# AsteriosPar/mmWave_MSc

Measured on AMD Instinct MI355X. Metric: scene_frames_per_sec, higher is better.
Workload: dtype f64

## Files before the change

mmwave_msc_amd/csrc/api_context.hip:

```cpp
#include <cmath>
#include <cstdarg>
#include <cstdio>
#include <new>

#include "mmw_ctx.hpp"
#include "mmw_kalman.hpp"

thread_local LaunchProf mmw::g_launch_prof;

static thread_local std::string g_last_error;

int fail(mmw_ctx *ctx, int code, const char *fmt, ...)
{
    char buf[512];
    va_list ap;
    va_start(ap, fmt);
    vsnprintf(buf, sizeof(buf), fmt, ap);
    va_end(ap);
    if (ctx) ctx->err = buf;
    g_last_error = buf;
    return code;
}

constexpr int kPerSceneMaxScenes = 512;
constexpr int kSideWorkerMinScenes = kPerSceneMaxScenes + 1;

static hipError_t create_side_streams(mmw_ctx *c)
{
    hipError_t e = hipStreamCreateWithFlags(&c->side_stream, hipStreamNonBlocking);
    if (e == hipSuccess) e = hipEventCreateWithFlags(&c->side_gate, hipEventDisableTiming);
    return e;
}

static int probe_one(mmw_ctx *c, hipStream_t side, hipStream_t other)
{
    const int polls = 1 << 12;
    if (hipMemsetAsync(c->d_probe, 0, 4 * sizeof(int32_t), c->stream) != hipSuccess || hipStreamSynchronize(c->stream) != hipSuccess) return -1;
    launch_probe_wait(c->d_probe, 0, polls, side);
    launch_probe_set(c->d_probe, other);
    if (hipStreamSynchronize(side) != hipSuccess || hipStreamSynchronize(other) != hipSuccess) return -1;
    int32_t w[4] = {0, 0, 0, 0};
    if (hipMemcpy(w, c->d_probe, sizeof(w), hipMemcpyDeviceToHost) != hipSuccess) return -1;
    return w[1] ? 1 : 0;
}
int probe_side_streams(mmw_ctx *c)
{
    int ok = probe_one(c, c->side_stream, c->stream);
    for (int attempt = 0; ok == 0 && attempt < 6; attempt++) {
        hipStream_t fresh = nullptr;
        if (hipStreamCreateWithFlags(&fresh, hipStreamNonBlocking) != hipSuccess) return -1;
        hipStreamSynchronize(c->side_stream);
        hipStreamDestroy(c->side_stream);
        c->side_stream = fresh;
        ok = probe_one(c, fresh, c->stream);
    }
    return ok;
}

static int check_create_args(const mmw_config *cfg, int32_t n_scenes, int32_t max_pts)
{
    if (n_scenes < 1 || max_pts < 1 || max_pts > MMW_MAX_PTS_LIMIT) return fail(nullptr, MMW_E_ARG, "mmw_create: n_scenes=%d max_pts=%d out of range (max_pts <= %d)", n_scenes, max_pts, MMW_MAX_PTS_LIMIT);
    if (cfg->fb_frames_batch < 0 || cfg->fb_frames_batch + 1 > MMW_RING_MAX) return fail(nullptr, MMW_E_ARG, "FB_FRAMES_BATCH must be in [0,%d]", MMW_RING_MAX - 1);
    if (cfg->dim_x != 9 && cfg->dim_x != 6) return fail(nullptr, MMW_E_ARG, "dim_x must be 9 (CONST_ACC_MODEL) or 6 (CONST_VEL_MODEL)");
    if (!(cfg->db_eps > 0.0) || cfg->db_min_samples < 1 || (cfg->seek_inner && !(cfg->db_inner_eps > 0.0)))
        return fail(nullptr, MMW_E_ARG, "DB_EPS%s must be > 0 and DB_MIN_SAMPLES_MIN >= 1 (sklearn's DBSCAN refuses anything else)", cfg->seek_inner ? " / DB_INNER_EPS" : "");
    const int um = (cfg->fb_frames_batch + 1) * max_pts;
    if (um > MMW_RING_MAX * MMW_MAX_PTS_LIMIT) return fail(nullptr, MMW_E_ARG, "ring*max_pts = %d exceeds %d", um, MMW_RING_MAX * MMW_MAX_PTS_LIMIT);
    return MMW_OK;
}

struct DevPlan { DevCfg dc; int fused_wanted, side_wanted, side_trusted, gate_side; };
static int derive_dev_cfg(const mmw_config *cfg, int32_t n_scenes, int32_t max_pts, DevPlan &plan)
{
    DevCfg &d = plan.dc;
    memset(&d, 0, sizeof(d));
    const int ring = cfg->fb_frames_batch + 1;
    d.ring = ring; d.db_min_samples = cfg->db_min_samples; d.tr_max_tracks = cfg->tr_max_tracks;
    d.kf_enable_est = cfg->kf_enable_est; d.model_min_input = cfg->model_min_input; d.dx = cfg->dim_x;
    d.ring_rows = cfg->ring_rows < 64 ? 64 : cfg->ring_rows;
    d.seek_inner = cfg->seek_inner ? 1 : 0;
    d.db_points_thres = cfg->db_points_thres; d.fb_frames_batch_static = cfg->fb_frames_batch_static;
    d.db_spread_thres = cfg->db_spread_thres; d.db_inner_eps = cfg->db_inner_eps;
    d.side_worker = (!d.seek_inner && (cfg->chain_side_stream > 0 || (cfg->chain_side_stream == 0 && n_scenes >= kSideWorkerMinScenes))) ? 1 : 0;
    if (d.seek_inner) {
        if (cfg->fb_frames_batch < 1 || cfg->fb_frames_batch_static < 1 || cfg->fb_frames_batch_static > ring)
            return fail(nullptr, MMW_E_ARG, "seek_inner: FB_FRAMES_BATCH and FB_FRAMES_BATCH_STATIC must be in [1, FB_FRAMES_BATCH + 1 = %d]", ring);
        if (d.ring_rows < ring * max_pts) d.ring_rows = ring * max_pts;
    }
    int cap = cfg->track_cap;
    if (cap <= 0) {
        const int ms = cfg->db_min_samples > 0 ? cfg->db_min_samples : 1;
        cap = (cfg->tr_max_tracks > 0 ? cfg->tr_max_tracks - 1 : 0) + (ring * max_pts) / ms + 1;
    }
    if (cap > MMW_TRACK_CAP_LIMIT) cap = MMW_TRACK_CAP_LIMIT;
    if (cap < 1) cap = 1;
    d.t_cap = cap; d.max_pts = max_pts; d.n_scenes = n_scenes;
    d.dense_min_units = cfg->kalman_dense_min_units == 0 ? (n_scenes <= kPerSceneMaxScenes ? 0x7fffffff : 1024)
                                                         : (cfg->kalman_dense_min_units < 0 ? 0x7fffffff : cfg->kalman_dense_min_units - 1);
    if (d.seek_inner) d.dense_min_units = 0x7fffffff;
    d.db_z_weight = cfg->db_z_weight; d.db_range_weight = cfg->db_range_weight; d.db_eps = cfg->db_eps;
    d.tr_lifetime_dynamic = cfg->tr_lifetime_dynamic; d.tr_lifetime_static = cfg->tr_lifetime_static;
    d.tr_vel_thres = cfg->tr_vel_thres; d.tr_gate = cfg->tr_gate; d.kf_q_std = cfg->kf_q_std; d.kf_p_init = cfg->kf_p_init;
    d.kf_group_disp_est_init = cfg->kf_group_disp_est_init; d.kf_a_n = cfg->kf_a_n; d.kf_est_pointnum = cfg->kf_est_pointnum;
    for (int i = 0; i < 6; i++) d.kf_spread_lim[i] = cfg->kf_spread_lim[i];
    d.kf_a_spr = cfg->kf_a_spr; d.intensity_mu = cfg->intensity_mu; d.intensity_std = cfg->intensity_std;
    d.s_height = cfg->s_height; d.tilt_cos = cfg->tilt_cos; d.tilt_sin = cfg->tilt_sin;
    d.m_x = cfg->m_x; d.m_y = cfg->m_y; d.m_z = cfg->m_z;
    d.fade_max = cfg->v_screen_fade_size_max; d.fade_min = cfg->v_screen_fade_size_min; d.fade_weight = cfg->v_screen_fade_weight;
    const size_t sl = scene_lds_bytes(d);
    const int per_cu = (sl <= 80 * 1024 && max_pts <= 512) ? 2 : (sl <= 160 * 1024 ? 1 : 0);
    const bool can = per_cu > 0 && !d.seek_inner && d.t_cap <= 63 && cfg->chain_side_stream <= 0;
    const bool want = cfg->fused_step > 0 || (cfg->fused_step == 0 && cfg->kalman_dense_min_units == 0 && n_scenes <= 256 * per_cu && n_scenes <= kPerSceneMaxScenes);
    plan.fused_wanted = d.fused = (can && want) ? 1 : 0;
    if (d.fused) { d.dense_min_units = 0x7fffffff; d.side_worker = 0; }
    plan.side_wanted = d.side_worker;
    plan.side_trusted = (d.side_worker && cfg->chain_side_stream == 2) ? 1 : 0;
    plan.gate_side = (d.side_worker && cfg->chain_side_stream == 3) ? 1 : 0;
    return MMW_OK;
}

static size_t trk_bytes(const DevCfg &d) { return (size_t)d.n_scenes * d.t_cap * sizeof(TrackRec); }
static size_t db_list_bytes(const DevCfg &d) { return 4 * (size_t)d.n_scenes * sizeof(int32_t); }
static size_t upd_list_bytes(const DevCfg &d) { return 2 * (size_t)kUpdShards * upd_region(d.n_scenes, d.t_cap) * sizeof(int32_t); }
static size_t inner_buf_bytes(const mmw_ctx *c) { return (size_t)c->dc.n_scenes * (size_t)(kInnerHdr + c->st.inner_cap) * sizeof(int32_t); }
constexpr size_t kStatAllocBytes = kStatBytes + (256 + 8192) * sizeof(unsigned long long);
constexpr size_t kDbCountBytes = 8 * sizeof(int32_t), kQBytes = kQWords * sizeof(int32_t), kSpcCountBytes = 2 * sizeof(int32_t), kUpdCountBytes = 2 * kUpdWords * sizeof(int32_t);

#define CREATE_FAIL(c, ...) do { mmw_destroy(c); return fail(nullptr, __VA_ARGS__); } while (0)

static int create_alloc(mmw_ctx *c)
{
    const DevCfg &d = c->dc;
#ifdef MMW_DIAG_POISON
#define MMW_POISON_FRESH(ptr, bytes) (void)hipMemsetAsync((void *)(ptr), 0xFF, (bytes), c->own_stream)
#else
#define MMW_POISON_FRESH(ptr, bytes) ((void)0)
#endif
    if (hipStreamCreateWithFlags(&c->own_stream, hipStreamNonBlocking) != hipSuccess) CREATE_FAIL(c, MMW_E_HIP, "hipStreamCreate failed");
    c->stream = c->own_stream;
#define ALLOC(ptr, bytes)                                                                                   \
    do {                                                                                                    \
        hipError_t e_ = hipMalloc((void **)&(ptr), (bytes));                                                \
        if (e_ != hipSuccess) { int rc = fail(nullptr, MMW_E_HIP, "hipMalloc(%zu) -> %s", (size_t)(bytes), hipGetErrorString(e_)); mmw_destroy(c); return rc; } \
        MMW_POISON_FRESH(ptr, bytes);                                                                       \
    } while (0)
    const size_t S = (size_t)d.n_scenes, cap = (size_t)d.t_cap;
    ALLOC(c->st.hdr, S * sizeof(SceneHdr));
    ALLOC(c->st.order, S * cap * sizeof(int32_t));
    ALLOC(c->st.trk, trk_bytes(d));
    ALLOC(c->st.trk_ring, S * cap * (size_t)d.ring * d.ring_rows * 8 * sizeof(double));
    ALLOC(c->st.g_ring, S * (size_t)d.ring * d.max_pts * 8 * sizeof(double));
    ALLOC(c->d_posture, MMW_NKP * sizeof(float));
    ALLOC(c->d_row_off, (S + 1) * sizeof(int32_t));
    ALLOC(c->st.stats, kStatAllocBytes);
    ALLOC(c->st.db_list, db_list_bytes(d));
    ALLOC(c->st.db_count, kDbCountBytes);
    ALLOC(c->st.q, kQBytes);
    ALLOC(c->d_probe, 4 * sizeof(int32_t));
    ALLOC(c->st.gate_buf, S * cap * kGateRec * sizeof(double));
    ALLOC(c->st.perm, 2 * S * sizeof(int32_t));
    ALLOC(c->st.upd_count, kUpdCountBytes);
    ALLOC(c->st.upd_list, upd_list_bytes(d));
    ALLOC(c->st.spc_count, kSpcCountBytes);
    ALLOC(c->st.spc_list, 4 * S * sizeof(int32_t));
    if (d.seek_inner) {
        c->st.inner_cap = 2 * inner_um(d);
        ALLOC(c->st.inner_buf, inner_buf_bytes(c));
    }
#undef ALLOC
#undef MMW_POISON_FRESH
    c->st.default_posture = c->d_posture;
    return MMW_OK;
}

static int create_init_device(mmw_ctx *c, int32_t n_scenes)
{
    const DevCfg &d = c->dc;
    const mmw_config *cfg = &c->cfg;
#ifdef MMW_MUTANT_NULL_STREAM_INIT
#define MMW_FILL0(ptr, bytes) hipMemset((ptr), 0, (bytes))
#else
#define MMW_FILL0(ptr, bytes) hipMemsetAsync((ptr), 0, (bytes), c->own_stream)
#endif
    if (hipMemcpyAsync(c->d_posture, cfg->default_posture, MMW_NKP * sizeof(float), hipMemcpyHostToDevice, c->own_stream) != hipSuccess ||
// ... 384 lines not shown
```

mmwave_msc_amd/csrc/k_track.hip:

```cpp
#include <cstdlib>

#include "mmw_device.hpp"
#include "mmw_math.hpp"
#include "mmw_cloud.hpp"
#include "mmw_kalman.hpp"
#include "mmw_assoc.hpp"
#include "mmw_launch.hpp"
#include "mmw_kernels.hpp"

namespace mmw {

#ifdef MMW_STAMPS
#define STAMP(k)                                                                              \
    do {                                                                                      \
        if (tid == 0) {                                                                       \
            const unsigned long long t_now = __builtin_amdgcn_s_memtime();                   \
            atomicAdd(&stats_slot(st, blockIdx.x)[8 + (k)], t_now - t_prev);                                    \
            t_prev = t_now;                                                                   \
        }                                                                                     \
    } while (0)
#else
#define STAMP(k)
#endif

struct TrackLds {
    double *p6;
    double *work;
    double *cen;
    unsigned short *cnt;
    int *cls_n;
    int *cls_off;
    long long *seg_dst;
    double *wmm;
    double *nest;
    int *ml;
    int *slot;
    int *slot2;
    int *misc;
};

template <bool WRITE>
__host__ __device__ __forceinline__ size_t track_lds_layout(const DevCfg &c, char *base, TrackLds *L)
{
    const int NP = c.max_pts, NB = (NP + 63) / 64, CLS = c.t_cap + 1;
    const int work_a = 0, work_b = 6 * (NP + kTilePad) + pw_max_leaves(NP) * 21;
    size_t off = 0;
#define CARVE(field, type, count)                            \
    if constexpr (WRITE) L->field = (type *)(base + off);    \
    off = align16(off + sizeof(type) * (size_t)(count));
    if constexpr (WRITE) L->p6 = (double *)(base + off);
    const int work_c = (12288 + 256 * 4 + 64) / 8;
    const int work_ab = work_a > work_b ? work_a : work_b;
    CARVE(work, double, work_ab > work_c ? work_ab : work_c)
    CARVE(cen, double, c.t_cap * 6)
    {
        const size_t base_off = off;
        CARVE(cnt, unsigned short, NB *CLS)
        CARVE(seg_dst, long long, CLS + 1)
        const size_t end_a = off;
        off = base_off;
        CARVE(wmm, double, kWaves * 24)
        CARVE(nest, double, c.t_cap)
        CARVE(slot2, int, c.t_cap)
        off = off > end_a ? off : end_a;
    }
    CARVE(cls_n, int, CLS)
    CARVE(cls_off, int, CLS + 1)
    CARVE(ml, int, ml_words(NP))
    CARVE(slot, int, c.t_cap)
    CARVE(misc, int, 16)
#undef CARVE
    return off;
}

size_t track_lds_bytes(const DevCfg &c)
{
    size_t b = track_lds_layout<false>(c, nullptr, nullptr);
    if (pred_in_track(c) && b < (size_t)16 * kPredScratch * sizeof(double)) b = (size_t)16 * kPredScratch * sizeof(double);
#ifdef MMW_STAMPS
    if (const char *x = getenv("MMW_DIAG_LDS_EXTRA")) b += (size_t)atoi(x);
#endif
    return b;
}

template <int PPT, bool INNER, bool PRED = false, bool F32 = false>
__global__ __launch_bounds__(kThreads, (PRED ? 2 : (PPT == 2 ? 5 : (PPT == 1 ? 4 : 3)))) void k_track(DevCfg cfg, DevState st, const void *__restrict__ pts_all,
                                                    const int32_t *__restrict__ n_pts, const double *__restrict__ dt_all,
                                                    int32_t *__restrict__ assoc_out, int32_t *__restrict__ db_n_out,
                                                    int32_t *__restrict__ db_labels_out, int UM_out, int parity)
{
    extern __shared__ __attribute__((aligned(16))) char lds_raw[];
    TrackLds L;
    track_lds_layout<true>(cfg, lds_raw, &L);

    const int s = st.perm[(size_t)parity * cfg.n_scenes + blockIdx.x];
    const int tid = threadIdx.x;
    const int lane = tid & 63, wave = tid >> 6;
    PROBE(19);
    WGTIME(0);
    const int role = (wave + s) & (kWaves - 1);
    const int NP = cfg.max_pts, CLS = cfg.t_cap + 1;
    const int NPs = NP + kTilePad;
    const int my_slot = tid < cfg.t_cap ? st.order[(size_t)s * cfg.t_cap + tid] : 0;
    const int n_raw = n_pts[s];
    SceneHdr *hdr = st.hdr + s;
    const double dt = dt_all[s];
    int T = hdr->n_tracks;
    double2 pr[PPT][4];
    {
        const void *frame = frame_of(pts_all, s, NP, F32);
#pragma unroll
        for (int q = 0; q < PPT; q++) {
            const int i = q * kThreads + tid;
            load_point_row<F32>(frame, i, i < NP, pr[q]);
        }
    }
    const int n = n_raw < 0 ? 0 : n_raw;
    if (tid == 0 && db_n_out) db_n_out[s] = -1;
    if (s == 0 && tid < 4) st.db_count[(parity ^ 1) * 4 + tid] = 0;
    if (s == 0 && tid >= 4 && tid < 7) st.q[(parity ^ 1) * 8 + (tid - 4)] = tid - 4 == kQHead ? q_tag(cfg.epoch + 1) : 0;
    if (s == 0 && tid >= 8 && tid < 11) st.q[kQBig + (parity ^ 1) * 8 + (tid - 8)] = tid - 8 == kQHead ? q_tag(cfg.epoch + 1) : 0;
    if (s == 0 && tid < kUpdWords) st.upd_count[(parity ^ 1) * kUpdWords + tid] = 0;
    if (s == 0 && tid == kThreads - 1) st.spc_count[parity ^ 1] = 0;
    if (!frame_reaches_track(n_raw, NP)) {
        if (tid == 0) frame_skipped(hdr, hdr->skipped, n_raw);
        return;
    }
    int32_t *order = st.order + (size_t)s * cfg.t_cap;
    TrackRec *trk = st.trk + (size_t)s * cfg.t_cap;
    const int Tin = T;
    int err = 0;
#ifdef MMW_STAMPS
    unsigned long long t_prev = __builtin_amdgcn_s_memtime();
#endif
    PROBE(16);
    if constexpr (PRED) {
        double *Wj = reinterpret_cast<double *>(lds_raw) + (size_t)(wave * 4 + (lane >> 4)) * kPredScratch;
        int perr = 0;
        for (int j0 = wave * 4; j0 < T; j0 += 4 * kWaves) {
            const int j = j0 + (lane >> 4);
            const bool live = j < T;
            TrackRec *rec = trk + (live ? order[j] : 0);
            if (cfg.dx == 9) predict_one_track<9>(cfg, st, rec, live, s, j, dt, Wj, lane, lane & 15, perr);
            else predict_one_track<6>(cfg, st, rec, live, s, j, dt, Wj, lane, lane & 15, perr);
        }
        PROBE(17);
        if (perr) atomicOr(&hdr->err, perr);
        __builtin_amdgcn_s_waitcnt(0x0F70);
        __builtin_amdgcn_fence(__ATOMIC_RELEASE, "workgroup");
        __syncthreads();
        __builtin_amdgcn_s_dcache_inv();
        __builtin_amdgcn_s_waitcnt(0xC07F);
        PROBE(18);
    }

    if (tid < cfg.t_cap) L.slot[tid] = my_slot;
    for (int j = tid + kThreads; j < cfg.t_cap; j += kThreads) L.slot[j] = order[j];
    if (tid == 0) { L.ml[0] = 0; L.ml[1] = 0; L.misc[15] = 0; }
    lds_barrier();
    STAMP(0);
    PROBE(0);

    double bestd[PPT];
    int bestj[PPT];
#pragma unroll
    for (int q = 0; q < PPT; q++) { bestd[q] = 0.0; bestj[q] = -1; }

    {
        const int su = __builtin_amdgcn_readfirstlane(s), Tu = __builtin_amdgcn_readfirstlane(T);
        gate_ptr gb = (gate_ptr)(st.gate_buf + (size_t)su * cfg.t_cap * kGateRec);
        if constexpr (PRED) {
            gb = gate_records_opaque(gb);
#ifndef MMW_DIAG_VGATE
            typedef const int __attribute__((address_space(4))) *line_ptr;
            const unsigned long long a0 = (unsigned long long)gb & ~63ULL;
            const int lines = (int)((((unsigned long long)gb + (unsigned long long)Tu * kGateRec * 8 + 63ULL) & ~63ULL) - a0) >> 6;
            line_ptr w = (line_ptr)a0;
            int acc = 0;
            for (int l0 = 0; l0 < lines; l0 += 16) {
                int t[16];
#pragma unroll
                for (int u = 0; u < 16; u++) { const int l = l0 + u < lines ? l0 + u : lines - 1; t[u] = w[l * 16]; }
#pragma unroll
                for (int u = 0; u < 16; u++) acc |= t[u];
            }
            asm volatile("" : : "s"(acc));
#endif
        }
        PROBE(32);
        for (int j = 0; j < Tu; j++) {
            if (j < 8) PROBE(33 + j);
            gate_ptr G = gb + j * kGateRec;
#pragma unroll
            for (int q = 0; q < PPT; q++) {
                const int i = q * kThreads + tid;
                if (q * kThreads < n) {
                    const double d = gate_distance(G, pr[q][0].x, pr[q][0].y, pr[q][1].x, pr[q][1].y, pr[q][2].x, pr[q][2].y);
                    gate_first_best(cfg, i < n, d, j, bestj[q], bestd[q]);
                }
            }
        }
    }
    STAMP(1);
    STAMP(2);
    PROBE(2);
    int gp_len, gp_skw, gp_s[MMW_RING_MAX], gp_n[MMW_RING_MAX];
    {
        const int NB = (n + 63) / 64;
        unsigned long long mybal[PPT];
        int sd_len = 0, sd_rs[MMW_RING_MAX] = {0, 0, 0, 0}, sd_size = cfg.ring;
        gp_len = 0; gp_skw = 0;
#pragma unroll
        for (int k = 0; k < MMW_RING_MAX; k++) { gp_s[k] = 0; gp_n[k] = 0; }
        if (tid < T) {
            const TrackRec *rec = trk + L.slot[tid];
            sd_len = rec->ring_len;
            if (INNER) sd_size = rec->inner & 255;
#pragma unroll
            for (int k = 0; k < MMW_RING_MAX; k++) sd_rs[k] = rec->ring_slot[k];
        } else if (tid == T) {
            sd_len = hdr->g_len;
            if (INNER && hdr_ring_size(hdr->skipped)) sd_size = hdr_ring_size(hdr->skipped);
#pragma unroll
            for (int k = 0; k < MMW_RING_MAX; k++) sd_rs[k] = hdr->g_slot[k];
        } else if (tid == kThreads - 1) {
            gp_len = hdr->g_len;
            gp_skw = hdr->skipped;
#pragma unroll
            for (int k = 0; k < MMW_RING_MAX; k++) { gp_s[k] = hdr->g_slot[k]; gp_n[k] = hdr->g_n[k]; }
        }
#pragma unroll
        for (int q = 0; q < PPT; q++) {
            const int i = q * kThreads + tid;
            const int blk = q * kWaves + wave;
            mybal[q] = 0;
            if (q == 0) PROBE(25);
            if (blk < NB) {
                const int cls = (i < n) ? bestj[q] + 1 : -1;
                if (i < n && assoc_out) assoc_out[(size_t)s * NP + i] = bestj[q];
                for (int c = 0; c <= T; c++) {
                    unsigned long long b = __ballot(cls == c);
                    if (cls == c) mybal[q] = b;
                    if (lane == 0) L.cnt[blk * CLS + c] = __popcll(b);
                }
            }
        }
        PROBE(26);
        lds_barrier();
        PROBE(27);
        for (int c = tid; c <= T; c += kThreads) {
            int t[PPT * kWaves];
#pragma unroll
            for (int b = 0; b < PPT * kWaves; b++) t[b] = b < NB ? L.cnt[b * CLS + c] : 0;
            int run = 0;
#pragma unroll
            for (int b = 0; b < PPT * kWaves; b++) { if (b < NB) L.cnt[b * CLS + c] = run; run += t[b]; }
            L.cls_n[c] = run;
        }
        lds_barrier();
        PROBE(28);
        for (int c = tid; c <= T + 1; c += kThreads) {
            int run = 0;
            for (int k = 0; k < c; k++) run += L.cls_n[k];
            L.cls_off[c] = run;
        }
        if (tid <= T) {
            int phys = sd_rs[0];
            if (INNER) {
                const int keepn = sd_len < sd_size - 1 ? sd_len : (sd_size - 1 > 0 ? sd_size - 1 : 0);
                const int want = sd_len > keepn ? sd_len - keepn - 1 : sd_len;
#pragma unroll
                for (int k = 1; k < MMW_RING_MAX; k++) if (k == want) phys = sd_rs[k];
            } else {
#pragma unroll
                for (int k = 1; k < MMW_RING_MAX; k++) if (sd_len < cfg.ring && k == sd_len) phys = sd_rs[k];
            }
            L.seg_dst[tid] = tid < T ? (((long long)s * cfg.t_cap + L.slot[tid]) * cfg.ring + phys) * (long long)cfg.ring_rows * 8
                                     : ((long long)s * cfg.ring + phys) * (long long)NP * 8;
        }
        lds_barrier();
        PROBE(30);
#pragma unroll
        for (int q = 0; q < PPT; q++) {
            const int i = q * kThreads + tid;
            if (i < n) {
                const int cls = bestj[q] + 1, blk = q * kWaves + wave;
                const int local = L.cnt[blk * CLS + cls] + __popcll(mybal[q] & lanemask_lt());
                const int pos = L.cls_off[cls] + local;
                L.p6[0 * NPs + pos] = pr[q][0].x; L.p6[1 * NPs + pos] = pr[q][0].y;
                L.p6[2 * NPs + pos] = pr[q][1].x; L.p6[3 * NPs + pos] = pr[q][1].y;
                L.p6[4 * NPs + pos] = pr[q][2].x; L.p6[5 * NPs + pos] = pr[q][2].y;
                if (cls == 0 || local < cfg.ring_rows) {
                    double *dst = (cls == 0 ? st.g_ring + L.seg_dst[T] : st.trk_ring + L.seg_dst[cls - 1]) + (size_t)local * 8;
                    double2 *d2 = reinterpret_cast<double2 *>(dst);
                    d2[0] = pr[q][0]; d2[1] = pr[q][1]; d2[2] = pr[q][2]; d2[3] = pr[q][3];
                }
                if (cls == 0) {
                    const int nfb = row_nonfinite_bits(pr[q]);
                    if (nfb) atomicOr(&L.misc[15], nfb);
                }
            }
        }
        PROBE(31);
        lds_barrier();
    }
    STAMP(3);
    if (tid == kThreads - 1) {
        int len = gp_len;
        const int gsz = (INNER && hdr_ring_size(gp_skw)) ? hdr_ring_size(gp_skw) : cfg.ring;
#pragma unroll
        for (int it = 0; it < MMW_RING_MAX; it++) {
            if (len >= gsz && len > 0) {
                const int first = gp_s[0];
#pragma unroll
                for (int k = 1; k < MMW_RING_MAX; k++) if (k < len) { gp_s[k - 1] = gp_s[k]; gp_n[k - 1] = gp_n[k]; }
#pragma unroll
                for (int k = 0; k < MMW_RING_MAX; k++) if (k == len - 1) gp_s[k] = first;
                len--;
            }
        }
        const int nun = L.cls_n[0];
        int phys = gp_s[0];
#pragma unroll
        for (int k = 1; k < MMW_RING_MAX; k++) if (k == len) phys = gp_s[k];
#pragma unroll
        for (int k = 0; k < MMW_RING_MAX; k++) if (k == len) gp_n[k] = nun;
        len++;
        int U = 0;
#pragma unroll
        for (int k = 0; k < MMW_RING_MAX; k++) { if (k >= len) gp_n[k] = 0; U += gp_n[k]; }
        int *gs = L.misc + 4, *gn = L.misc + 8;
#pragma unroll
        for (int k = 0; k < MMW_RING_MAX; k++) { gs[k] = gp_s[k]; gn[k] = gp_n[k]; hdr->g_slot[k] = gp_s[k]; hdr->g_n[k] = gp_n[k]; }
        hdr->g_len = len;
        hdr->db_u = U;
        L.misc[1] = phys;
        L.misc[3] = len;
        L.misc[13] = U;
        const int nff = nf_ring_flags(gp_skw, phys, L.misc[15]);
        int live = 0;
#pragma unroll
        for (int k = 0; k < MMW_RING_MAX; k++) if (k < len) live |= (nff >> (2 * gp_s[k])) & 3;
        L.misc[15] = nff | (live << 8);
    }
    PROBE(3);

    auto finish = [&](int j, int m, int nj, double sum, double mn, double mx, double old, double ne_old, TrackRec *rec) {
        if (nj == 0) {
            if (m == 0) rec->lifetime += dt;
            return;
        }
        const double cen = sum / (double)nj;
        L.cen[j * 6 + m] = cen;
        rec->centroid[m] = cen;
        rec->minv[m] = mn;
        rec->maxv[m] = mx;
        rec->spread[m] = spread_estimate(cfg, m, nj, mn, mx, old);
        if (m == 0) {
            if (nj > 128) {
                int cnt = 0;
                pw_for_each_leaf<kPwDepth>(0, nj, [&](int, int) { cnt++; });
                const int first = atomicAdd(&L.ml[0], cnt), c = atomicAdd(&L.ml[1], 1);
                int *lf = L.ml + 2 + first * 3, *cl = L.ml + 2 + 3 * pw_max_leaves(NP);
                cl[c * 2] = j; cl[c * 2 + 1] = first;
                int k = 0;
                pw_for_each_leaf<kPwDepth>(0, nj, [&](int o, int len) { lf[k * 3] = j; lf[k * 3 + 1] = o; lf[k * 3 + 2] = len; k++; });
            }
            rec->lifetime = 0.0;
            rec->point_num = nj;
            const double ne = point_num_estimate(cfg, nj, ne_old);
            rec->n_est = ne;
            L.nest[j] = ne;
        }
    };
    if (T <= 10) {
        double mn = __longlong_as_double(0x7ff0000000000000LL), mx = -mn, old = 0.0, ne_old = 0.0;
        int fg = -1;
        if (role == 0) {
            const int grp = lane / 6, m = lane - grp * 6, j = grp;
            const bool valid = lane < 60 && j < T;
            const int nj = valid ? L.cls_n[j + 1] : 0, off = valid ? L.cls_off[j + 1] : 0;
            if (nj > 0) {
                const double *col = L.p6 + m * NPs + off;
                double sum = 0.0;
                int r = 0;
                double v[8], w[8];
                if (nj >= 8) {
#pragma unroll
                    for (int u = 0; u < 8; u++) v[u] = col[u];
                    for (r = 8; r + 8 <= nj; r += 8) {
#pragma unroll
                        for (int u = 0; u < 8; u++) w[u] = col[r + u];
#pragma unroll
                        for (int u = 0; u < 8; u++) sum += v[u];
#pragma unroll
                        for (int u = 0; u < 8; u++) v[u] = w[u];
                    }
#pragma unroll
                    for (int u = 0; u < 8; u++) sum += v[u];
                }
                {
                    const int left = nj - r;
#pragma unroll
                    for (int u = 0; u < 7; u++) v[u] = (u < left) ? col[r + u] : 0.0;
#pragma unroll
                    for (int u = 0; u < 7; u++) if (u < left) sum += v[u];
                }
                L.cen[j * 6 + m] = sum;
            }
        } else {
            int lg = 5;
            while (lg > 0 && 6 * T * (1 << lg) > 192) lg--;
            const int task = (role - 1) * 64 + lane, g = task >> lg, slice = task & ((1 << lg) - 1);
            const int j = g / 6, m = g - j * 6;
            const bool valid = g < 6 * T;
            const int nj = valid ? L.cls_n[j + 1] : 0, off = valid ? L.cls_off[j + 1] : 0;
            TrackRec *rec = trk + L.slot[valid ? j : 0];
            if (valid && slice == 0) {
                fg = g;
                if (nj > 0) {
                    old = rec->spread[m];
                    if (m == 0) ne_old = rec->n_est;
                }
            }
            if (nj > 0) {
                const double *col = L.p6 + m * NPs + off;
// ... 27 lines not shown
            const int fj = fg / 6, fn = L.cls_n[fj + 1];
            finish(fj, fg - fj * 6, fn, fn > 0 ? L.cen[fg] : 0.0, mn, mx, old, ne_old, trk + L.slot[fj]);
        }
    } else {
        for (int jb = 0; jb < T; jb += 2 * kWaves) {
            const bool grpA = lane < 12, grpB = lane >= 16;
            const int pi = grpA ? lane : (grpB ? (lane - 16) >> 2 : 0), slice = (lane - 16) & 3;
            const int jj = pi / 6, m = pi - jj * 6, j = jb + wave * 2 + jj;
            const bool valid = j < T && (grpA || grpB);
            const int nj = valid ? L.cls_n[j + 1] : 0, off = valid ? L.cls_off[j + 1] : 0;
            TrackRec *rec = trk + L.slot[valid ? j : 0];
            const double *col = L.p6 + m * NPs + off;
            double old = 0.0, ne_old = 0.0, sum = 0.0;
            PROBE(20);
            if (grpA && nj > 0) {
                old = rec->spread[m];
                if (m == 0) ne_old = rec->n_est;
                int r = 0;
                double v[8], w[8];
                if (nj >= 8) {
#pragma unroll
                    for (int u = 0; u < 8; u++) v[u] = col[u];
                    for (r = 8; r + 8 <= nj; r += 8) {
#pragma unroll
                        for (int u = 0; u < 8; u++) w[u] = col[r + u];
#pragma unroll
                        for (int u = 0; u < 8; u++) sum += v[u];
#pragma unroll
                        for (int u = 0; u < 8; u++) v[u] = w[u];
                    }
#pragma unroll
                    for (int u = 0; u < 8; u++) sum += v[u];
                }
                {
                    const int left = nj - r;
    #pragma unroll
                    for (int u = 0; u < 7; u++) v[u] = (u < left) ? col[r + u] : 0.0;
    #pragma unroll
                    for (int u = 0; u < 7; u++) if (u < left) sum += v[u];
                }
            }
            PROBE(21);
            double mn = __longlong_as_double(0x7ff0000000000000LL), mx = -mn;
            if (grpB && nj > 0) {
                const int r0 = (nj * slice) >> 2, r1 = (nj * (slice + 1)) >> 2;
                if (r0 < r1) { mn = col[r0]; mx = mn; }
                int r = r0 + 1;
                for (; r + 8 <= r1; r += 8) {
                    double v[8];
    #pragma unroll
                    for (int u = 0; u < 8; u++) v[u] = col[r + u];
    #pragma unroll
                    for (int u = 0; u < 8; u++) { mn = v[u] < mn ? v[u] : mn; mx = v[u] > mx ? v[u] : mx; }
                }
                {
                    const int left = r1 - r;
                    double v[7];
    #pragma unroll
                    for (int u = 0; u < 7; u++) v[u] = (u < left) ? col[r + u] : mn;
    #pragma unroll
                    for (int u = 0; u < 7; u++) if (u < left) { mn = v[u] < mn ? v[u] : mn; mx = v[u] > mx ? v[u] : mx; }
                }
            }
            PROBE(22);
    #pragma unroll
            for (int d = 1; d <= 2; d <<= 1) {
                const double tn = __shfl_down(mn, d), tx = __shfl_down(mx, d);
                mn = tn < mn ? tn : mn;
                mx = tx > mx ? tx : mx;
            }
            double *wmm = L.wmm + wave * 24;
            if (grpB && slice == 0) { wmm[pi * 2] = mn; wmm[pi * 2 + 1] = mx; }
            wave_sync();
            PROBE(23);
            if (grpA && valid) finish(j, m, nj, sum, nj > 0 ? wmm[pi * 2] : 0.0, nj > 0 ? wmm[pi * 2 + 1] : 0.0, old, ne_old, rec);
            wave_sync();
        }
    }
    PROBE(24);
    lds_barrier();
    STAMP(4);
    PROBE(4);
    double sx = 0.0, sy = 0.0, sz = 0.0;
    {
        const int Ucl = L.misc[13], nun = L.cls_n[0];
        if (Ucl <= 256 && tid < Ucl) {
            const int old_n = Ucl - nun;
            if (tid >= old_n) {
                const int k = tid - old_n;
                sx = L.p6[0 * NPs + k]; sy = L.p6[1 * NPs + k]; sz = L.p6[2 * NPs + k];
            } else {
                const int *gs = L.misc + 4, *gn = L.misc + 8;
                int f = 0, base = 0;
#pragma unroll
                for (int k = 0; k < MMW_RING_MAX - 1; k++) if (tid >= base + gn[f] && f < L.misc[3] - 2) { base += gn[f]; f++; }
                const double *r = st.g_ring + ((size_t)s * cfg.ring + gs[f]) * (size_t)NP * 8 + (size_t)(tid - base) * 8;
                const double2 a = *reinterpret_cast<const double2 *>(r);
                sx = a.x; sy = a.y; sz = r[2];
            }
        }
    }
    for (int j = kThreads - 1 - tid; j < T; j += kThreads) {
        const int nj = L.cls_n[j + 1];
        if (nj == 0 && INNER) trk[L.slot[j]].inner &= 255;
        if (nj > 0) {
            TrackRec *rec = trk + L.slot[j];
            const int rsize = INNER ? (rec->inner & 255) : cfg.ring;
            rec->is_static = centroid_is_static(cfg, L.cen[j * 6 + 3], L.cen[j * 6 + 4], L.cen[j * 6 + 5]);
            int len = rec->ring_len;
            int rn[MMW_RING_MAX], rs[MMW_RING_MAX];
#pragma unroll
            for (int k = 0; k < MMW_RING_MAX; k++) { rn[k] = rec->ring_n[k]; rs[k] = rec->ring_slot[k]; }
            while (len >= rsize && len > 0) {
                const int first = rs[0];
#pragma unroll
                for (int k = 1; k < MMW_RING_MAX; k++) if (k < len) { rs[k - 1] = rs[k]; rn[k - 1] = rn[k]; }
#pragma unroll
                for (int k = 0; k < MMW_RING_MAX; k++) if (k == len - 1) rs[k] = first;
                len--;
            }
#pragma unroll
            for (int k = 0; k < MMW_RING_MAX; k++) if (k == len) rn[k] = nj;
#pragma unroll
            for (int k = 0; k < MMW_RING_MAX; k++) { rec->ring_n[k] = rn[k]; rec->ring_slot[k] = rs[k]; }
            rec->ring_len = len + 1;
            if (INNER) rec->inner = rsize | kInnerTouched;
        }
    }
    {
        PROBE(10);
        double *leafsum = L.work + 6 * NPs;
        const int nleaf = L.ml[0], ncloud = L.ml[1];
        const int *lf = L.ml + 2, *cl = L.ml + 2 + 3 * pw_max_leaves(NP);
        auto blend = [&](TrackRec *rec, int a, int b, double res, int nj, double g_ab, double g_ba, double ne) {
            const double D = res / (double)nj;
            if (ne == 0.0) { err |= ERR_DIVZERO; return; }
            const double al = (double)nj / ne;
            rec->gd[a * 6 + b] = (1 - al) * g_ab + al * D;
            if (a != b) rec->gd[b * 6 + a] = (1 - al) * g_ba + al * D;
        };
        for (int it = tid; it < (T + nleaf) * 21; it += kThreads) {
            const int u = it / 21;
            int a, b;
            disp_entry(it - u * 21, a, b);
            const bool direct = u < T;
            const int j = direct ? u : lf[(u - T) * 3];
            const int nj = L.cls_n[j + 1];
            if (direct && (nj == 0 || nj > 128)) continue;
            const int off = L.cls_off[j + 1] + (direct ? 0 : lf[(u - T) * 3 + 1]), len = direct ? nj : lf[(u - T) * 3 + 2];
            TrackRec *rec = trk + L.slot[j];
            PROBE(11);
            double g_ab = 0.0, g_ba = 0.0, ne = 1.0;
            if (direct) { g_ab = rec->gd[a * 6 + b]; g_ba = rec->gd[b * 6 + a]; ne = L.nest[j]; }
            const double res = pw_leaf(L.p6 + a * NPs + off, L.p6 + b * NPs + off, L.cen[j * 6 + a], L.cen[j * 6 + b], len);
            PROBE(12);
            if (direct) blend(rec, a, b, res, nj, g_ab, g_ba, ne);
            else leafsum[(u - T) * 21 + (it - u * 21)] = res;
        }
        PROBE(13);
        if (ncloud > 0) {
            lds_barrier();
            PROBE(14);
            for (int it = tid; it < ncloud * 21; it += kThreads) {
                const int c = it / 21, e = it - c * 21;
                int a, b;
                disp_entry(e, a, b);
                const int j = cl[c * 2], nj = L.cls_n[j + 1];
                TrackRec *rec = trk + L.slot[j];
                const double g_ab = rec->gd[a * 6 + b], g_ba = rec->gd[b * 6 + a], ne = L.nest[j];
                int idx = 0;
                const double res = pw_combine<kPwDepth>(nj, leafsum + cl[c * 2 + 1] * 21 + e, 21, idx);
                blend(rec, a, b, res, nj, g_ab, g_ba, ne);
            }
        }
        PROBE(15);
    }
    STAMP(5);
    __syncthreads();
    {
        int *grid = reinterpret_cast<int *>(reinterpret_cast<char *>(L.work) + 4096);
        for (int i = tid; i < kCloudGrid; i += kThreads) grid[i] = 0;
        if (tid == 0) { grid[kCloudGrid] = 0; grid[kCloudGrid + 1] = 0; L.misc[12] = 0; }
    }
    STAMP(6);

    if (role == 0) {
        const bool have = lane < T;
        bool keep = false;
        int sl = 0;
        if (have) {
            sl = L.slot[lane];
            const TrackRec *rec = trk + sl;
            const double lim = rec->is_static ? cfg.tr_lifetime_static : cfg.tr_lifetime_dynamic;
            keep = !(rec->lifetime > lim);
        }
        const unsigned long long kb = __ballot(have && keep), db = __ballot(have && !keep);
        const int nk = __popcll(kb);
        if (have) {
            const int pos = keep ? __popcll(kb & lanemask_lt()) : nk + __popcll(db & lanemask_lt());
            L.slot2[pos] = sl;
        }
        if (lane == 0) L.misc[0] = nk;
    }
    lds_barrier();
    {
        const int Told = T;
        T = L.misc[0];
        for (int j = tid; j < Told; j += kThreads) { L.slot[j] = L.slot2[j]; order[j] = L.slot2[j]; }
    }
    lds_barrier();
    PROBE(6);
    STAMP(7);

    const int upd_units = cfg.n_scenes * kalman_waves_per_scene(cfg.tr_max_tracks);
    const bool upd_on = tracks_dense(cfg, kalman_waves_per_scene(cfg.tr_max_tracks));
    const int upd_sh = (int)blockIdx.x % upd_shards(upd_units);
    int upd_pos = -1;
    STAMP(8);
    if (tid == 0) {
        const int U = L.misc[13];
        hdr->n_tracks = T;
        hdr->n_upd = T;
        const int nfw = L.misc[15];
        hdr->skipped = (INNER ? (hdr->skipped & (kSkipRingMask << kSkipRingShift)) : 0) | ((nfw & kSkipNfMask) << kSkipNfShift);
        if (T > 0 && upd_on) upd_pos = atomicAdd(&st.upd_count[parity * kUpdWords + upd_sh], T);
        bool need = U > 0 && T < cfg.tr_max_tracks;
        const int nfe = nf_error_of(nfw >> 8);
        if (need && nfe) {
            if (INNER && cfg.seek_inner) hdr->need_db = 2 | (nfe << 2);
            else {
                err |= nfe;
                hdr->need_db = 0;
                if (db_n_out) db_n_out[s] = kDbRaised;
            }
            need = false;
        } else
            hdr->need_db = need ? 1 : 0;
        L.misc[2] = need ? U : 0;
    }
    if (err) atomicOr(&hdr->err, err);
    STAMP(9);
    PROBE(8);
    lds_barrier();
    const int Udb = L.misc[2];
    if (Udb > 0) {
        bool listed = true;
        int *grid = reinterpret_cast<int *>(reinterpret_cast<char *>(L.work) + 4096);
        unsigned long long *mm = reinterpret_cast<unsigned long long *>(grid + kCloudGrid);
        if (Udb <= 256) {
            listed = !cloud_cells_prove_no_core(cfg, Udb, sx, sy, sz, mm, &L.misc[12], grid);
            if (listed) {
                float4 *P4 = reinterpret_cast<float4 *>(L.work);
                int *pcnt = reinterpret_cast<int *>(reinterpret_cast<char *>(L.work) + 12288);
                unsigned long long *mm2 = reinterpret_cast<unsigned long long *>(pcnt + 256);
                listed = !cloud_pairs_prove_no_core_xyz<kThreads>(cfg, Udb, sx, sy, sz, P4, pcnt, mm2, &L.misc[14]);
            }
        } else {
            const int *gs = L.misc + 4, *gn = L.misc + 8;
            const int nfr = L.misc[3], big = 0x7fffffff;
            RowSrc src;
            src.gb = st.g_ring + (size_t)s * cfg.ring * (size_t)NP * 8;
            src.stride = (size_t)NP * 8;
            src.slots = (unsigned)gs[0] | ((unsigned)gs[1] << 8) | ((unsigned)gs[2] << 16) | ((unsigned)gs[3] << 24);
            src.c1 = nfr > 1 ? gn[0] : big;
            src.c2 = nfr > 2 ? gn[0] + gn[1] : big;
            src.c3 = nfr > 3 ? gn[0] + gn[1] + gn[2] : big;
            listed = !cloud_cells_prove_no_core_rows(cfg, src, Udb, mm, &L.misc[12], grid);
        }
        if (listed) {
            const int cls = Udb <= 256 ? (Udb >= kEarlyU && cfg.side_worker ? 0 : 3) : (Udb <= kBigCloudMax ? 1 : 2);
            const bool live = cls == 0 || (cls == 1 && cfg.big_live);
            if (live) __syncthreads();
            if (tid == 0) {
                int32_t *cnt = cls >= 2 ? st.db_count + parity * 4 + cls : st.q + cls * kQBig + parity * 8 + kQCount;
                const int pos = atomicAdd(cnt, 1);
                int32_t *e = st.db_list + (size_t)cls * cfg.n_scenes + pos;
                if (cls >= 2) *e = s;
                else if (live) __hip_atomic_store(e, s + 1, __ATOMIC_RELEASE, __HIP_MEMORY_SCOPE_AGENT);
                else __hip_atomic_store(e, s + 1, __ATOMIC_RELAXED, __HIP_MEMORY_SCOPE_AGENT);
            }
        } else {
            cloud_finish_empty(st, hdr, s, Udb, UM_out, db_labels_out, db_n_out);
        }
    }
    PROBE(9);
    STAMP(10);
    if (tid == 0 && st.stats) {
        int ring_rows = 0;
        for (int j = 0; j < Tin; j++) ring_rows += min(L.cls_n[j + 1], cfg.ring_rows);
        step_account(stats_slot(st, s), F32, n, Tin, L.cls_n[0], ring_rows);
    }
    if (tid < 64) {
        const int pos = __builtin_amdgcn_readfirstlane(upd_pos);
        if (pos >= 0 && tid < T) st.upd_list[((size_t)parity * kUpdShards + upd_sh) * upd_region(cfg.n_scenes, cfg.t_cap) + pos + tid] = upd_pack(s, tid, L.slot[tid]);
    }
    WGTIME(1);
}

template <int PPT, bool F32>
// ... 61 lines not shown
```

mmwave_msc_amd/csrc/mmw_device.hpp:

```cpp
#pragma once

#include <hip/hip_runtime.h>
#include <stdint.h>

#include "../../include/mmw.h"
#include "mmw_uidlist.hpp"

namespace mmw {

constexpr int kThreads = 256;
constexpr int kWaves = kThreads / 64;
constexpr int kGateChunk = 16;
constexpr int kGateRec = 44;
constexpr int kLeafSize = 30;
constexpr int kSkNeighbors = 5;
constexpr int kMaxLeaves = 32;
constexpr int kBigCloudMax = 30 * 64;
constexpr int kMaxNodes = 63;

enum : int { ERR_SINGULAR = 1, ERR_DIVZERO = 2, ERR_CAPACITY = 4, ERR_BADCOUNT = 8, ERR_NONFINITE_NAN = 16, ERR_NONFINITE_INF = 32 };
constexpr int kDbRaised = -2;

struct DevCfg {
    int32_t ring;
    int32_t db_min_samples;
    int32_t tr_max_tracks;
    int32_t kf_enable_est;
    int32_t model_min_input;
    int32_t dx;
    int32_t ring_rows;
    int32_t t_cap;
    int32_t max_pts;
    int32_t n_scenes;
    int32_t dense_min_units;
    int32_t seek_inner;
    int32_t db_points_thres, fb_frames_batch_static;
    int32_t big_live;
    int32_t fused;
    int32_t epoch;
    int32_t var_ring, side_worker;
    double db_spread_thres, db_inner_eps;
    double db_z_weight, db_range_weight, db_eps;
    double tr_lifetime_dynamic, tr_lifetime_static, tr_vel_thres, tr_gate;
    double kf_q_std, kf_p_init, kf_group_disp_est_init, kf_a_n, kf_est_pointnum;
    double kf_spread_lim[6];
    double kf_a_spr;
    double intensity_mu, intensity_std;
    double s_height, tilt_cos, tilt_sin;
    double m_x, m_y, m_z, fade_max, fade_min, fade_weight;
};

struct SceneHdr {
    int32_t n_tracks;
    int32_t g_len;
    int32_t g_n[MMW_RING_MAX];
    int32_t g_slot[MMW_RING_MAX];
    int32_t need_db;
    int32_t err;
    int32_t db_u;
    int32_t next_uid;
    int32_t n_upd;
    int32_t skipped;
};
static_assert(sizeof(SceneHdr) == 64, "SceneHdr");
constexpr int kSkipRingShift = 8, kSkipRingMask = 255, kSkipNfShift = 16, kSkipNfMask = 255;
__host__ __device__ inline int hdr_ring_size(int skipped) { return (skipped >> kSkipRingShift) & kSkipRingMask; }
__device__ __forceinline__ int row_nonfinite_bits(const double2 (&r)[4])
{
    constexpr int kNanInf = 0x3 | 0x4 | 0x200;
    bool any = false;
#pragma unroll
    for (int u = 0; u < 4; u++) any = any || __builtin_amdgcn_class(r[u].x, kNanInf) || __builtin_amdgcn_class(r[u].y, kNanInf);
    if (!any) return 0;
    bool nan = false, inf = false;
#pragma unroll
    for (int u = 0; u < 4; u++) {
        nan = nan || __builtin_amdgcn_class(r[u].x, 0x3) || __builtin_amdgcn_class(r[u].y, 0x3);
        inf = inf || __builtin_amdgcn_class(r[u].x, 0x204) || __builtin_amdgcn_class(r[u].y, 0x204);
    }
    return (nan ? 1 : 0) | (inf ? 2 : 0);
}
__host__ __device__ inline int nf_flags_with(int flags, int phys, int frame_bits) { return (flags & ~(3 << (2 * phys))) | ((frame_bits & 3) << (2 * phys)); }
__host__ __device__ inline int nf_error_of(int bits) { return (bits & 1) ? ERR_NONFINITE_NAN : ((bits & 2) ? ERR_NONFINITE_INF : 0); }
__host__ __device__ inline double xyz_q_divisor(unsigned q) { return q <= 62 ? (double)(1ull << q) : (q == 63 ? -9223372036854775808.0 : 0.0); }

constexpr int kUartBuf = MMW_UART_BUFFER;
struct UartScene {
    double t_last;
    double half_bins;
    double doppler_res;
    int32_t len;
    int32_t reserved;
};
static_assert(sizeof(UartScene) == 32, "UartScene");
struct UartState {
    uint8_t *buf;
    UartScene *scene;
};
struct UartLogWord {
    double t;
    double range_scale;
    uint32_t frame;
    int32_t count;
    uint32_t head;
    int32_t fresh;
};
static_assert(sizeof(UartLogWord) == 32, "UartLogWord");
struct UartLog {
    UartLogWord *word;
    uint8_t *obj;
};

struct TrackRec {
    double x[9];
    double P[81];
    double centroid[6];
    double minv[6];
    double maxv[6];
    double spread[6];
    double gd[36];
    double n_est;
    double lifetime;
    int32_t point_num;
// ... 122 lines not shown
```

Measured before the change: 18.25 million.

## Skip clustering and lifetime pruning when every track receives points and track set is full

Adds a settle path in the track kernel: when every live track gets at least one point in the frame, the lifetime-expiry compaction pass is skipped, and when the track count also equals the maximum, the unassigned-point clustering and new-track creation work is skipped. In that case the block writes the header fields and the Kalman update list directly, then returns early. The aim is to remove the DBSCAN and spawn work and barriers for frames with a full, fully-fed track set. This relies on the assumption that seen tracks cannot expire, which holds only for non-negative lifetime limits and is gated on that; it adds a ballot and an atomic on the common path.

```diff
diff --git a/mmwave_msc_amd/csrc/api_context.hip b/mmwave_msc_amd/csrc/api_context.hip
--- a/mmwave_msc_amd/csrc/api_context.hip
+++ b/mmwave_msc_amd/csrc/api_context.hip
@@ -100,6 +100,7 @@
     if (d.seek_inner) d.dense_min_units = 0x7fffffff;
     d.db_z_weight = cfg->db_z_weight; d.db_range_weight = cfg->db_range_weight; d.db_eps = cfg->db_eps;
     d.tr_lifetime_dynamic = cfg->tr_lifetime_dynamic; d.tr_lifetime_static = cfg->tr_lifetime_static;
+    d.settle_ok = (cfg->tr_lifetime_dynamic >= 0.0 && cfg->tr_lifetime_static >= 0.0) ? 1 : 0;
     d.tr_vel_thres = cfg->tr_vel_thres; d.tr_gate = cfg->tr_gate; d.kf_q_std = cfg->kf_q_std; d.kf_p_init = cfg->kf_p_init;
     d.kf_group_disp_est_init = cfg->kf_group_disp_est_init; d.kf_a_n = cfg->kf_a_n; d.kf_est_pointnum = cfg->kf_est_pointnum;
     for (int i = 0; i < 6; i++) d.kf_spread_lim[i] = cfg->kf_spread_lim[i];
diff --git a/mmwave_msc_amd/csrc/k_track.hip b/mmwave_msc_amd/csrc/k_track.hip
--- a/mmwave_msc_amd/csrc/k_track.hip
+++ b/mmwave_msc_amd/csrc/k_track.hip
@@ -38,6 +38,40 @@
     int *slot2;
     int *misc;
 };
+
+constexpr int kAllSeen = 1, kSettled = 2;
+#ifdef MMW_DIAG_NO_SETTLE
+constexpr bool kSettleBuilt = false;
+#else
+constexpr bool kSettleBuilt = true;
+#endif
+__device__ __forceinline__ int settle_word(const DevCfg &cfg, int T, unsigned long long seen)
+{
+    if (!cfg.settle_ok || T < 1 || __popcll(seen) != T) return 0;
+    return kAllSeen | (T >= cfg.tr_max_tracks ? kSettled : 0);
+}
+template <bool INNER>
+__device__ __forceinline__ int ring_push_slot(const DevCfg &cfg, int len, int size, int rs0, int rs1, int rs2, int rs3)
+{
+    static_assert(MMW_RING_MAX == 4, "ring_push_slot takes the ring's four slots by value");
+    int phys = rs0;
+    if (INNER) {
+        const int keepn = len < size - 1 ? len : (size - 1 > 0 ? size - 1 : 0);
+        const int want = len > keepn ? len - keepn - 1 : len;
+        phys = want == 1 ? rs1 : phys;
+        phys = want == 2 ? rs2 : phys;
+        phys = want == 3 ? rs3 : phys;
+    } else if (len < cfg.ring) {
+        phys = len == 1 ? rs1 : phys;
+        phys = len == 2 ? rs2 : phys;
+        phys = len == 3 ? rs3 : phys;
+    }
+    return phys;
+}
+__device__ __forceinline__ int upd_shard_of(const DevCfg &cfg)
+{
+    return (int)blockIdx.x % upd_shards(cfg.n_scenes * kalman_waves_per_scene(cfg.tr_max_tracks));
+}
 
 template <bool WRITE>
 __host__ __device__ __forceinline__ size_t track_lds_layout(const DevCfg &c, char *base, TrackLds *L)
@@ -204,7 +238,9 @@
     STAMP(1);
     STAMP(2);
     PROBE(2);
+    constexpr bool kSettle = kSettleBuilt && !INNER;
     int gp_len, gp_skw, gp_s[MMW_RING_MAX], gp_n[MMW_RING_MAX];
+    int settle = 0, settled_pos = -1;
     {
         const int NB = (n + 63) / 64;
         unsigned long long mybal[PPT];
@@ -259,22 +295,19 @@
         }
         lds_barrier();
         PROBE(28);
+        if constexpr (kSettle) {
+            const int n_mine = lane < T ? L.cls_n[lane + 1] : 0;
+            settle = settle_word(cfg, T, __ballot(n_mine > 0));
+            if ((settle & kSettled) && role == 0 && lane == 0 && tracks_dense(cfg, kalman_waves_per_scene(cfg.tr_max_tracks)))
+                settled_pos = atomicAdd(&st.upd_count[parity * kUpdWords + upd_shard_of(cfg)], T);
+        }
         for (int c = tid; c <= T + 1; c += kThreads) {
             int run = 0;
             for (int k = 0; k < c; k++) run += L.cls_n[k];
             L.cls_off[c] = run;
         }
         if (tid <= T) {
-            int phys = sd_rs[0];
-            if (INNER) {
-                const int keepn = sd_len < sd_size - 1 ? sd_len : (sd_size - 1 > 0 ? sd_size - 1 : 0);
-                const int want = sd_len > keepn ? sd_len - keepn - 1 : sd_len;
-#pragma unroll
-                for (int k = 1; k < MMW_RING_MAX; k++) if (k == want) phys = sd_rs[k];
-            } else {
-#pragma unroll
-                for (int k = 1; k < MMW_RING_MAX; k++) if (sd_len < cfg.ring && k == sd_len) phys = sd_rs[k];
-            }
+            const int phys = ring_push_slot<INNER>(cfg, sd_len, sd_size, sd_rs[0], sd_rs[1], sd_rs[2], sd_rs[3]);
             L.seg_dst[tid] = tid < T ? (((long long)s * cfg.t_cap + L.slot[tid]) * cfg.ring + phys) * (long long)cfg.ring_rows * 8
                                      : ((long long)s * cfg.ring + phys) * (long long)NP * 8;
         }
@@ -342,6 +375,11 @@
 #pragma unroll
         for (int k = 0; k < MMW_RING_MAX; k++) if (k < len) live |= (nff >> (2 * gp_s[k])) & 3;
         L.misc[15] = nff | (live << 8);
+        if (settle & kSettled) {
+            hdr->n_upd = T;
+            hdr->skipped = (nff & kSkipNfMask) << kSkipNfShift;
+            hdr->need_db = 0;
+        }
     }
     PROBE(3);
 
@@ -535,7 +573,7 @@
     STAMP(4);
     PROBE(4);
     double sx = 0.0, sy = 0.0, sz = 0.0;
-    {
+    if (!(settle & kSettled)) {
         const int Ucl = L.misc[13], nun = L.cls_n[0];
         if (Ucl <= 256 && tid < Ucl) {
             const int old_n = Ucl - nun;
@@ -629,6 +667,20 @@
         PROBE(15);
     }
     STAMP(5);
+    if (settle & kSettled) {
+        if (err) atomicOr(&hdr->err, err);
+        if (tid == 0 && st.stats) {
+            int ring_rows = 0;
+            for (int j = 0; j < Tin; j++) ring_rows += min(L.cls_n[j + 1], cfg.ring_rows);
+            step_account(stats_slot(st, s), F32, n, Tin, L.cls_n[0], ring_rows);
+        }
+        if (role == 0) {
+            const int pos = __builtin_amdgcn_readfirstlane(settled_pos);
+            if (pos >= 0 && lane < T) st.upd_list[((size_t)parity * kUpdShards + upd_shard_of(cfg)) * upd_region(cfg.n_scenes, cfg.t_cap) + pos + lane] = upd_pack(s, lane, L.slot[lane]);
+        }
+        WGTIME(1);
+        return;
+    }
     __syncthreads();
     {
         int *grid = reinterpret_cast<int *>(reinterpret_cast<char *>(L.work) + 4096);
@@ -637,37 +689,38 @@
     }
     STAMP(6);
 
-    if (role == 0) {
-        const bool have = lane < T;
-        bool keep = false;
-        int sl = 0;
-        if (have) {
-            sl = L.slot[lane];
-            const TrackRec *rec = trk + sl;
-            const double lim = rec->is_static ? cfg.tr_lifetime_static : cfg.tr_lifetime_dynamic;
-            keep = !(rec->lifetime > lim);
-        }
-        const unsigned long long kb = __ballot(have && keep), db = __ballot(have && !keep);
-        const int nk = __popcll(kb);
-        if (have) {
-            const int pos = keep ? __popcll(kb & lanemask_lt()) : nk + __popcll(db & lanemask_lt());
-            L.slot2[pos] = sl;
-        }
-        if (lane == 0) L.misc[0] = nk;
-    }
-    lds_barrier();
-    {
-        const int Told = T;
-        T = L.misc[0];
-        for (int j = tid; j < Told; j += kThreads) { L.slot[j] = L.slot2[j]; order[j] = L.slot2[j]; }
-    }
-    lds_barrier();
+    if (!(settle & kAllSeen)) {
+        if (role == 0) {
+            const bool have = lane < T;
+            bool keep = false;
+            int sl = 0;
+            if (have) {
+                sl = L.slot[lane];
+                const TrackRec *rec = trk + sl;
+                const double lim = rec->is_static ? cfg.tr_lifetime_static : cfg.tr_lifetime_dynamic;
+                keep = !(rec->lifetime > lim);
+            }
+            const unsigned long long kb = __ballot(have && keep), db = __ballot(have && !keep);
+            const int nk = __popcll(kb);
+            if (have) {
+                const int pos = keep ? __popcll(kb & lanemask_lt()) : nk + __popcll(db & lanemask_lt());
+                L.slot2[pos] = sl;
+            }
+            if (lane == 0) L.misc[0] = nk;
+        }
+        lds_barrier();
+        {
+            const int Told = T;
+            T = L.misc[0];
+            for (int j = tid; j < Told; j += kThreads) { L.slot[j] = L.slot2[j]; order[j] = L.slot2[j]; }
+        }
+        lds_barrier();
+    }
     PROBE(6);
     STAMP(7);
 
-    const int upd_units = cfg.n_scenes * kalman_waves_per_scene(cfg.tr_max_tracks);
     const bool upd_on = tracks_dense(cfg, kalman_waves_per_scene(cfg.tr_max_tracks));
-    const int upd_sh = (int)blockIdx.x % upd_shards(upd_units);
+    const int upd_sh = upd_shard_of(cfg);
     int upd_pos = -1;
     STAMP(8);
     if (tid == 0) {
diff --git a/mmwave_msc_amd/csrc/mmw_device.hpp b/mmwave_msc_amd/csrc/mmw_device.hpp
--- a/mmwave_msc_amd/csrc/mmw_device.hpp
+++ b/mmwave_msc_amd/csrc/mmw_device.hpp
@@ -39,6 +39,7 @@
     int32_t fused;
     int32_t epoch;
     int32_t var_ring, side_worker;
+    int32_t settle_ok;
     double db_spread_thres, db_inner_eps;
     double db_z_weight, db_range_weight, db_eps;
     double tr_lifetime_dynamic, tr_lifetime_static, tr_vel_thres, tr_gate;
```

After: 18.38 million, median of 6. About the same (+0.7%).
